# RomanJuranek/librectify

Hardware: AMD Instinct MI355X
Metric: Mpix/s end-to-end (detect+VP) on 4K frames, batch call of 64 frames, 5 in flight (higher is better)
Workload: dtype f32

## Files before the change

include/librectify_amd.h:

```cpp
#pragma once
#include <math.h>
#include <stddef.h>
#include <stdint.h>

#include "librectify.h"

#if defined(__GNUC__)
#pragma GCC visibility push(default)
#endif

#ifdef __cplusplus
using librectify::ImageTransform;
using librectify::LineSegment;
using librectify::Point;
using librectify::RectificationConfig;
extern "C" {
#endif

typedef struct lr_context lr_context;
enum lr_pixel_format { LR_PIX_U8 = 0, LR_PIX_U8X3 = 1, LR_PIX_F32 = 2 };

int lr_context_create(int device, lr_context** out);
void lr_context_destroy(lr_context* ctx);
void lr_release_thread_context(void);
// ... 349 lines not shown
int lr_stage_seeds(lr_context* ctx, int* n_seeds);
int lr_stage_flood(lr_context* ctx, int* n_components);
int lr_stage_fit(lr_context* ctx, LineSegment* out, int capacity, int* n_lines);

enum lr_buffer_id {
    LR_BUF_DX = 0,
    LR_BUF_DY = 1,
    LR_BUF_DMASK = 2,
    LR_BUF_LABEL = 3,
    LR_BUF_SEED_IDX = 4,
    LR_BUF_SEED_BIN = 5,
    LR_BUF_SEED_THR = 6,
    LR_BUF_MAXMAG = 7,
    LR_BUF_SEED_SIZE = 8,
    LR_BUF_SEED_REC = 9,
};
int lr_download(lr_context* ctx, int buffer_id, void* dst, size_t bytes);

enum lr_stage_id {
    LR_T_UPLOAD = 0,
    LR_T_FILTER = 1,
    LR_T_SEEDS = 2,
    LR_T_FLOOD = 3,
    LR_T_FIT = 4,
    LR_T_RANSAC = 5,
    LR_T_TOTAL = 6,
    LR_T_FILTER_KERNEL = 7,
    LR_T_COUNT = 8,
};
int lr_stage_times(lr_context* ctx, float* ms, int count);
// ... 33 lines not shown
```

librectify_amd/__init__.py:

```python
import collections
import ctypes as C
import os

import numpy as np

_HERE = os.path.dirname(os.path.abspath(__file__))
LIB_PATH = os.path.join(_HERE, "librectify_amd.so")

LINE_DTYPE = np.dtype(
    [("x1", "<f4"), ("y1", "<f4"), ("x2", "<f4"), ("y2", "<f4"), ("weight", "<f4"), ("err", "<f4"), ("group_id", "<i4")]
)


class Point(C.Structure):
    _fields_ = [("x", C.c_float), ("y", C.c_float), ("z", C.c_float)]


class ImageTransform(C.Structure):
    _fields_ = [
        ("width", C.c_int),
        ("height", C.c_int),
        ("top_left", Point),
        ("top_right", Point),
        ("bottom_left", Point),
# ... 30 lines not shown

class DrawLinesArgs(C.Structure):
    _fields_ = [("lines", C.c_void_p), ("n_lines", C.c_size_t), ("frames", C.c_void_p), ("H", C.c_void_p)]


class JpegArgs(C.Structure):
    _fields_ = [("frames", C.c_void_p), ("sizes", C.c_void_p)]


class JpegDecodeArgs(C.Structure):
    _fields_ = [("h_src", C.c_void_p), ("frames", C.c_void_p), ("info", C.c_void_p)]


BUF_DX, BUF_DY, BUF_DMASK, BUF_LABEL, BUF_SEED_IDX, BUF_SEED_BIN, BUF_SEED_THR, BUF_MAXMAG, BUF_SEED_SIZE = range(9)
BUF_SEED_REC = 9
T_UPLOAD, T_FILTER, T_SEEDS, T_FLOOD, T_FIT, T_RANSAC, T_TOTAL, T_FILTER_KERNEL, T_COUNT = range(9)
PIX_U8, PIX_U8X3, PIX_F32 = range(3)
WARP_PREPARE = 0x100
WARP_PACKED = 0x200
WARP_RAGGED = 0x800
WARP_LINES = 0x1000
JPEG_OPTIMIZE = 0x10
WARP_JPEG = 0x2000
WARP_CUBIC = 0x8000
JPEG_SCALED = 0x80000
JPEG_ANY_SAMPLING = 0x20000
WARP_JPEG_DECODE = 0x4000
WARP_BORDER = 0x40000
BORDER_CONSTANT, BORDER_REPLICATE, BORDER_REFLECT, BORDER_REFLECT_101 = 0, 1, 2, 4
WARP_LENS = 0x100000
# ... 912 lines not shown
        h, w = self.shape
        if buf in (BUF_DX, BUF_DY):
            a = np.zeros((h, w), np.float32)
        elif buf == BUF_DMASK:
            a = np.zeros((h, w), np.uint8)
        elif buf == BUF_LABEL:
            a = np.zeros((h, w), np.int32)
        elif buf in (BUF_SEED_IDX, BUF_SEED_BIN, BUF_SEED_SIZE):
            a = np.zeros(self.n_seeds, np.int32)
        elif buf == BUF_SEED_THR:
            a = np.zeros(self.n_seeds, np.float32)
        elif buf == BUF_MAXMAG:
            a = np.zeros(1, np.float32)
        elif buf == BUF_SEED_REC:
            a = np.zeros((self.n_seeds, 4), np.uint32)
        else:
            raise ValueError(buf)
        if a.nbytes:
            _check(lib().lr_download(self._h, buf, _ptr(a), a.nbytes))
        return a

    def stage_times(self):
        t = np.zeros(T_COUNT, np.float32)
        _check(lib().lr_stage_times(self._h, _ptr(t), T_COUNT))
        return t

    def stage_times_partial(self):
        ms = C.c_float(0)
        _check(lib().lr_filter_kernel_ms(self._h, C.byref(ms)))
        return ms.value
# ... 945 lines not shown
```

librectify_amd/csrc/api.cpp:

```cpp
#include <algorithm>
#include <cstdio>
#include <cstdlib>
#include <cstring>
#include <memory>
#include <new>
#include <stdexcept>
#include <string>

#include "context.h"
#include "host.h"

using namespace lramd;

namespace {

struct CtxDeleter {
    void operator()(lr_context* c) const { ctx_destroy(c); }
};

std::unique_ptr<lr_context, CtxDeleter>& thread_context_slot() {
    thread_local std::unique_ptr<lr_context, CtxDeleter> ctx;
    return ctx;
}

// ... 451 lines not shown
    try {
        const size_t npix = (size_t)ctx->w * ctx->h;
        const void* src = nullptr;
        size_t have = 0;
        switch (buffer_id) {
            case LR_BUF_DX: src = ctx->ws.dx; have = npix * 4; break;
            case LR_BUF_DY: src = ctx->ws.dy; have = npix * 4; break;
            case LR_BUF_DMASK: src = ctx->ws.dmask; have = npix; break;
            case LR_BUF_LABEL: src = ctx->ws.label; have = npix * 4; break;
            case LR_BUF_SEED_IDX: src = ctx->ws.seed_idx; have = (size_t)ctx->n_seeds * 4; break;
            case LR_BUF_SEED_BIN: src = ctx->ws.seed_bin; have = (size_t)ctx->n_seeds * 4; break;
            case LR_BUF_SEED_THR: src = ctx->ws.seed_thr; have = (size_t)ctx->n_seeds * 4; break;
            case LR_BUF_MAXMAG: src = ctx->maxmag; have = 4; break;
            case LR_BUF_SEED_SIZE: src = ctx->ws.seed_size; have = (size_t)ctx->n_seeds * 4; break;
            case LR_BUF_SEED_REC: src = ctx->ws.seed_rec; have = (size_t)ctx->n_seeds * 16; break;
            default: set_error("lr_download: unknown buffer id"); return 1;
        }
        if (buffer_id == LR_BUF_DMASK && ctx->dmask_consumed) {
            set_error("lr_download: LR_BUF_DMASK was consumed by lr_stage_flood (labelled pixels are cleared); download it after lr_stage_filter");
            return 1;
        }
        if (bytes > have) {
            set_error("lr_download: request larger than the buffer");
            return 1;
        }
        LR_HIP(hipSetDevice(ctx->device));
        LR_HIP(hipStreamSynchronize(ctx->stream));
        LR_HIP(hipMemcpy(dst, src, bytes, hipMemcpyDeviceToHost));
        return 0;
    } catch (...) {
// ... 83 lines not shown

int lr_refine_lines(lr_context* ctx, const LineSegment* in, int n, LineSegment* out, int* n_out) {
    try {
        std::vector<LineSegment> v(in, in + n);
        if (ctx_refine(ctx, v)) return 1;
        std::memcpy(out, v.data(), v.size() * sizeof(LineSegment));
        *n_out = (int)v.size();
        return 0;
    } catch (...) {
        return guard_fail("lr_refine_lines");
    }
}

void lr_set_estimator(lr_context* ctx, int kind, int param) {
    ctx->opt.estimator = kind;
    if (kind == 3) ctx->opt.cht_d = param > 0 ? param : 128;
    else ctx->opt.prosac_T_N = param;
}

int lr_estimate_line_pencils_cht(lr_context* ctx, LineSegment* lines, int n, int max_models, float inlier_deg,
                                 float garbage_deg, int d, float* models3, int* n_models, uint32_t* peak_cells,
                                 uint64_t* votes) {
    try {
        std::vector<LineSegment> v(lines, lines + n);
        ChtTrace tr;
        if (ctx_estimate_line_pencils_cht(ctx, v, max_models, inlier_deg, garbage_deg, d, &tr)) return 1;
        std::memcpy(lines, v.data(), sizeof(LineSegment) * (size_t)n);
        for (size_t k = 0; k < tr.models.size(); ++k) {
            if (models3) {
                models3[3 * k + 0] = tr.models[k].x;
// ... 87 lines not shown
```

librectify_amd/csrc/common.h:

```cpp
#pragma once
#include <hip/hip_runtime.h>

#include <cstdint>
#include <string>

#include "../../include/librectify_amd.h"

namespace lramd {

constexpr float kEps = 1e-6f;
constexpr int kMaxModels = 4;
constexpr int kMaxPeelModels = 5;
constexpr float kInlierDeg = 2.0f;
constexpr float kGarbageDeg = 4.0f;
constexpr int kRansacMaxIter = 10000;
constexpr int kEdgeKernelSize = 2;
constexpr float kEdgeKernelSigma = 1.0f;
constexpr int kSeedDist = 2;
constexpr float kSeedRatio = 0.95f;
constexpr float kTraceTolerance = 0.25f;
constexpr float kLineMaxErr = 2.0f;
constexpr float kLineMinLength = 5.f;
constexpr int kComponentMinSize = 5;
constexpr int kBins = 8;
// ... 186 lines not shown
    uint32_t scheduled = 0;
};
constexpr int kFloodCtrlWords = 56;
int flood_enqueue(const FloodBuffers& B, const FloodFrame& F, FloodProgress* P, uint32_t* h_ctrl, hipStream_t s);
int flood_finish(const FloodBuffers& B, const FloodFrame& F, FloodProgress* P, uint32_t* h_ctrl, int* rounds_out,
                 uint32_t* tiers_out ,
                 bool* extra, hipStream_t s);

size_t fit_temp_bytes(size_t max_pixels, uint32_t max_segments);
struct HugeSort {
    uint32_t* tab = nullptr;
    uint32_t* list = nullptr;
    uint32_t* jobs = nullptr;
    uint32_t max = 0;
};
int launch_component_offsets(const int32_t* seed_size, const uint32_t* d_n_seeds, uint32_t seed_cap, int min_size,
                             uint32_t* comp_rank, uint32_t* comp_seed, uint32_t* comp_off,
                             uint32_t* totals , uint32_t* large_list, uint32_t large_cap,
                             uint32_t* n_large, void* temp, size_t temp_bytes, uint32_t frame_tag, uint32_t* cursor, const HugeSort& hs,
                             hipStream_t s);
int launch_component_scatter(const uint32_t* label, size_t npix, const uint32_t* comp_rank, const uint32_t* comp_off,
                             uint32_t* cursor, uint32_t* px, const HugeSort& hs, uint32_t* n_large, bool with_huge, hipStream_t s);
int launch_component_sort(const uint32_t* px_in, uint32_t* px_out, const uint32_t* comp_off, const uint32_t* d_n_comp,
                          uint32_t comp_cap, const uint32_t* large_list, uint32_t large_cap, const uint32_t* n_large,
                          uint32_t* scratch, const uint32_t* cursor, const HugeSort& hs, bool with_huge, hipStream_t s);
int launch_fit(const uint32_t* px_sorted, const uint32_t* px_unsorted, const uint32_t* comp_off, const uint32_t* comp_seed, const uint32_t* d_n_comp,
               uint32_t comp_cap, const int32_t* seed_bin, const float* dx, const float* dy, int w, BinTrig trig,
               float* scratch_w, LineSegment* out, const uint32_t* cursor, const HugeSort& hs, const uint32_t* n_large, bool with_huge,
               hipStream_t s);

struct PencilSoA {
    const float* ax;
    const float* ay;
// ... 18 lines not shown
    float* len;
    float* hx;
    float* hy;
    float* hz;
    uint32_t* orig;
    PencilSoA soa() const { return PencilSoA{ax, ay, dx, dy, len, hx, hy, hz}; }
};
enum {
    kGcLines = 0,
    kGcRemaining = 1,
    kGcRound = 2,
    kGcActive = 3,
    kGcBestIter0 = 4,
    kGcWords = 8,
};
int launch_filter_lines(const LineSegment* raw, const uint32_t* d_n_raw, uint32_t raw_cap, float min_length,
                        LineSegment* out, uint32_t* gctl, float* gnorm, const PencilTable* all, const PencilTable* round0,
                        hipStream_t s);
int launch_lines_bbox(LineSegment* lines, uint32_t n, uint32_t* gctl, float* gnorm, hipStream_t s);
int launch_pencil_model(const LineSegment* lines, const uint32_t* gctl, const float* gnorm, PencilTable all,
                        PencilTable round0, uint32_t line_cap, hipStream_t s);
int launch_peel(PencilTable cur, PencilTable nxt, PencilTable all, unsigned long long* best_slots, uint64_t seed,
                float tol, float garbage_tol, int max_models, uint32_t* gctl, float* stage4 ,
                LineSegment* lines, float* models,
                const uint32_t* counts, uint32_t cap_lines, void* gather_block ,
                hipStream_t s);
int launch_cht_accumulate(PencilSoA m, uint32_t n, int d, unsigned long long* acc, hipStream_t s);
int launch_cht_votes(PencilSoA m, const uint32_t* idx, uint32_t n, int d, unsigned long long* acc, bool subtract,
                     unsigned long long* n_votes, hipStream_t s);
int launch_cht_peak(const unsigned long long* acc, int d, uint32_t* out3, hipStream_t s);
int launch_refine_pairs(const void* seg, uint32_t n, void* edges, uint32_t* n_edges, uint32_t cap, hipStream_t s);
// ... 10 lines not shown
```

librectify_amd/csrc/context.h:

```cpp
#pragma once
#include <atomic>
#include <functional>
#include <memory>
#include <mutex>
#include <vector>

#include "buffers.h"
#include "common.h"
#include "vp_host.h"

namespace lramd {
struct StagingCrew;

struct Settings {
    uint64_t ransac_seed = 0;
    int ransac_iters = kRansacMaxIter;
    int estimator = 0;
    int prosac_T_N = -1;
    int cht_d = 128;
    int batch_streams = 5;
    int flood_mode = 1;
    bool flood_giant_step = true;
    bool flood_jit = true;
    bool flood_partial = true;
    bool flood_log_sweep = false;
    bool flood_logs = true;
    bool flood_staged = false;
    bool timing_on = false;
};


struct Workspace {
    size_t cap_pix = 0;
    int cap_tiles = 0;
    DeviceBuffer<float> dx, dy;
    DeviceBuffer<uint8_t> dmask;
    DeviceBuffer<uint64_t> cand;
    DeviceBuffer<uint32_t> cand_count, tile_max;
    DeviceBuffer<uint32_t> tile_pass;
    DeviceBuffer<uint32_t> tile_off;
    DeviceBuffer<uint64_t> keys_a, keys_b;
    DeviceBuffer<int32_t> seed_idx, seed_bin;
// ... 254 lines not shown
```

librectify_amd/csrc/frame.hip:

```cpp
#include "host.h"

#include <cstdio>
#include <cstdlib>
#include <cstring>

namespace lramd {


namespace {

uint32_t round_up(uint32_t v, uint32_t m) { return (v + m - 1) / m * m; }

uint32_t initial_seed_cap(size_t npix) {
    return (uint32_t)std::min<size_t>(npix, std::max<size_t>(round_up((uint32_t)(npix / 32), 1024), 4096));
}

uint32_t line_cap_for(const lr_context* c) {
    return (uint32_t)std::min<size_t>(c->seed_cap, c->ws.cap_pix / 6 + 16);
}


PencilTable table_of(lr_context* c, int which) {
    const size_t cl = c->cap_glines;
    float* b = c->d_tables + (size_t)which * 8 * cl;
// ... 171 lines not shown
    c->flood_hold_hint = c->flood_tiers[3] != 0 && c->flood_tiers[8] >= 16;
    constexpr uint32_t kStagedKeep = 64;
    c->flood_staged_hint = c->flood_tiers[14] != 0 && (!c->flood_staged_hint || c->flood_tiers[0] >= kStagedKeep);
    c->flood_staged_streak = c->flood_staged_hint ? c->flood_staged_streak + 1 : 0;
    if (c->flood_staged_streak >= 16) {
        c->flood_staged_hint = false;
        c->flood_staged_streak = 0;
    }
    if (c->flood_staged_hint) c->flood_hold_hint = false;

    c->flood_rounds_hint = std::max(std::max(c->flood_rounds + 2, 6), c->flood_rounds_hint - 1);
    c->flood_rounds_last = c->flood_rounds;
    return 0;
}

int enqueue_fit(lr_context* c) {
    const size_t npix = (size_t)c->w * c->h;
    const uint32_t comp_cap = line_cap_for(c);
    const bool with_huge = !(c->opt.flood_mode != 0 && c->flood_prog.sizes_known && c->flood_prog.max_flood <= (1u << 14));
    if (launch_component_offsets(c->ws.seed_size, c->d_counts + kCntSeeds, c->seed_cap, kComponentMinSize, c->ws.comp_rank,
                                 c->ws.comp_seed, c->ws.comp_off, c->d_counts + kCntComp, c->ws.comp_large,
                                 (uint32_t)(c->ws.cap_pix / 64 + 16), c->d_counts + kCntLarge, c->ws.temp, c->ws.temp.cap(), ++c->fit_tag ? c->fit_tag : ++c->fit_tag, c->ws.cursor,
                                 with_huge ? c->ws.huge : HugeSort{}, c->stream))
        return 1;
    if (launch_component_scatter(c->ws.label, npix, c->ws.comp_rank, c->ws.comp_off, c->ws.cursor, c->ws.px_a, c->ws.huge, c->d_counts + kCntLarge, with_huge,
                                 c->stream))
        return 1;
    if (launch_component_sort(c->ws.px_a, c->ws.px_b, c->ws.comp_off, c->d_counts + kCntComp, comp_cap, c->ws.comp_large,
                              (uint32_t)(c->ws.cap_pix / 64 + 16), c->d_counts + kCntLarge, reinterpret_cast<uint32_t*>(c->ws.keys_b.get()),
                              c->ws.cursor, c->ws.huge, with_huge, c->stream))
        return 1;
    static const bool fit_debug = std::getenv("LIBRECTIFY_FIT_DEBUG") != nullptr;
    if (fit_debug) {
        uint32_t cnt[16];
        LR_HIP(hipStreamSynchronize(c->stream));
        LR_HIP(hipMemcpy(cnt, c->d_counts, sizeof(cnt), hipMemcpyDeviceToHost));
        std::fprintf(stderr, "fit: with_huge %d (sizes known %d, largest flood %u); seeds %u comps %u px %u; lists: %u of 65..1024 px, %u longer, %u huge in %u buckets; counter %u\n",
                     (int)with_huge, (int)c->flood_prog.sizes_known, c->flood_prog.max_flood, cnt[0], cnt[1], cnt[2], cnt[4], cnt[5], cnt[6], cnt[7], cnt[10]);
        const uint32_t nj = std::min<uint32_t>(cnt[7], 6);
        std::vector<uint32_t> jobs(4 * nj + 4);
        if (nj) LR_HIP(hipMemcpy(jobs.data(), c->ws.huge.jobs, nj * 16, hipMemcpyDeviceToHost));
        for (uint32_t j = 0; j < nj; ++j) std::fprintf(stderr, "   bucket job %u: start %u, %u px, table word %u\n", j, jobs[4 * j], jobs[4 * j + 1], jobs[4 * j + 2]);
    }
    if (launch_fit(c->ws.px_b, c->ws.px_a, c->ws.comp_off, c->ws.comp_seed, c->d_counts + kCntComp, comp_cap, c->ws.seed_bin, c->ws.dx, c->ws.dy, c->w,
                   c->trig, c->ws.scratch_w, c->ws.d_lines, c->ws.cursor, c->ws.huge, c->d_counts + kCntLarge, with_huge, c->stream))
        return 1;
    if (c->opt.timing_on) LR_HIP(hipEventRecord(c->ev[4], c->stream));
    return 0;
}

}

int enqueue_groups(lr_context* c, uint32_t line_cap, int max_models, float inlier_deg, float garbage_deg, int n_iter,
                   uint64_t seed, bool model_done, bool gather) {
    if (max_models > kMaxPeelModels) {
        set_error("estimate_line_pencils: max_models above " + std::to_string(kMaxPeelModels) + " (the reference uses 4, config.h:25)");
        return 1;
    }
    const float tol = cos_threshold(inlier_deg), garbage_tol = cos_threshold(garbage_deg);
// ... 23 lines not shown
    (void)hipEventElapsedTime(&ms, c->ev[0], c->ev[1]);
    c->stage_ms[LR_T_FILTER] = ms;
    c->stage_ms[LR_T_FILTER_KERNEL] = ms;
    (void)hipEventElapsedTime(&ms, c->ev[1], c->ev[2]);
    c->stage_ms[LR_T_SEEDS] = ms;
    (void)hipEventElapsedTime(&ms, c->ev[2], c->ev[3]);
    c->stage_ms[LR_T_FLOOD] = ms;
    (void)hipEventElapsedTime(&ms, c->ev[3], c->ev[4]);
    c->stage_ms[LR_T_FIT] = ms;
    if (with_groups) {
        (void)hipEventElapsedTime(&ms, c->ev[5], c->ev[6]);
        c->stage_ms[LR_T_RANSAC] = ms;
        (void)hipEventElapsedTime(&ms, c->ev[0], c->ev[6]);
        c->stage_ms[LR_T_TOTAL] = ms;
    }
}

void adapt_seed_cap(lr_context* c, uint32_t n_seeds) {
    const size_t npix = (size_t)c->w * c->h;
    if (n_seeds > c->seed_cap)
        c->seed_cap = (uint32_t)std::min<size_t>(npix, std::max<uint32_t>(4096, round_up(n_seeds * 2u, 1024)));
    else if (n_seeds < c->seed_cap / 3 || n_seeds > c->seed_cap / 5 * 4)
        c->seed_cap = (uint32_t)std::min<size_t>(npix, std::max<uint32_t>(4096, round_up(n_seeds + n_seeds / 2, 1024)));
}

}

struct TimingOn {
    lr_context* c;
    bool was;
// ... 68 lines not shown
    return 0;
}

int ctx_detect(lr_context* c, const float* d_image, int w, int h, int stride, std::vector<LineSegment>& raw) {
    if (ctx_stage_filter(c, d_image, w, h, stride)) return 1;
    if (ctx_stage_seeds(c)) return 1;
    if (ctx_stage_flood(c)) return 1;
    return ctx_stage_fit(c, raw);
}

int run_frame(lr_context* c, const void* d_image, int format, int w, int h, int stride, float min_length, bool refine,
              std::vector<LineSegment>& out, bool filter_enqueued) {
    out.clear();
    const double t_begin = now_ms();
    const bool fused = !refine && c->opt.estimator == 0;
    const int n_iter = c->opt.ransac_iters;
    auto groups_after_fit = [&]() -> int {
        const uint32_t lc = line_cap_for(c);
        if (ensure_group_capacity(c, lc)) return 1;
        if (ensure_result_block(c, std::max<size_t>(c->res_lines_cap, 4096))) return 1;
        if (c->opt.timing_on) LR_HIP(hipEventRecord(c->ev[5], c->stream));
        const PencilTable all = table_of(c, 0), round0 = table_of(c, 1);
        if (launch_filter_lines(c->ws.d_lines, c->d_counts + kCntComp, lc, min_length, c->d_flines, c->d_gctl, c->d_gnorm, &all, &round0,
                                c->stream))
            return 1;
        static_assert(kMaxModels >= 1 && kGcWords == 8 && kResHeaderBytes == 256, "the last peeling round carries the result block (peel_kernel)");
        if (enqueue_groups(c, lc, kMaxModels, kInlierDeg, kGarbageDeg, n_iter, c->opt.ransac_seed, true, true)) return 1;
        if (c->opt.timing_on) LR_HIP(hipEventRecord(c->ev[6], c->stream));
        return 0;
    };
    auto after_fit = [&]() -> int {
        if (fused) return groups_after_fit();
        LR_HIP(hipMemcpyAsync(c->h_counts, c->d_counts, 8 * sizeof(uint32_t), hipMemcpyDeviceToHost, c->stream));
        return 0;
    };
    c->frame_laps = 0;
    for (int attempt = 0;; ++attempt) {
        c->frame_laps += 1;
        if (!(filter_enqueued && attempt == 0) && enqueue_filter(c, d_image, format, w, h, stride)) return 1;
        if (enqueue_seeds(c)) return 1;
        if (enqueue_flood(c)) return 1;
        if (enqueue_fit(c)) return 1;
        if (after_fit()) return 1;
        const double t_enq = now_ms();
        const double t_pre = now_ms();
        if (c->sleep_in_wait) {
            LR_HIP(hipEventRecord(c->ev_wait, c->stream));
            LR_HIP(hipEventSynchronize(c->ev_wait));
        } else {
            LR_HIP(hipStreamSynchronize(c->stream));
        }
        c->host_ms[0] = t_enq - t_begin;
        c->host_ms[1] = t_pre - t_enq;
        c->host_ms[2] = now_ms() - t_pre;
        const uint32_t* cnt = fused ? reinterpret_cast<const uint32_t*>(c->h_res.get()) : c->h_counts.get();
        c->n_seeds = cnt[kCntSeeds];
        if (c->n_seeds <= c->seed_cap) break;
        if (attempt > 0) {
            set_error("seed count exceeds the sort capacity twice");
            return 1;
        }
        adapt_seed_cap(c, c->n_seeds);
    }
    bool extra = false;
    if (finish_flood(c, &extra)) return 1;
    if (extra) {
        c->frame_laps += 1;
        if (enqueue_fit(c)) return 1;
        if (after_fit()) return 1;
        LR_HIP(hipStreamSynchronize(c->stream));
    }
    const uint32_t* cnt = fused ? reinterpret_cast<const uint32_t*>(c->h_res.get()) : c->h_counts.get();
    c->n_comp = cnt[kCntComp];
    c->n_px = cnt[kCntPx];
    adapt_seed_cap(c, c->n_seeds);
    c->stage_valid[0] = c->stage_valid[1] = false;
    c->stage_valid[2] = c->stage_valid[3] = true;
    if (fused) {
        const uint32_t* gctl = reinterpret_cast<const uint32_t*>(c->h_res + 32);
        const size_t n = gctl[kGcLines];
        out.resize(n);
        const size_t have = std::min<size_t>(n, c->res_lines_cap);
        if (have) std::memcpy(out.data(), c->h_res + kResHeaderBytes, have * sizeof(LineSegment));
        if (n > have) {
            LR_HIP(hipMemcpyAsync(out.data() + have, c->d_flines + have, (n - have) * sizeof(LineSegment),
                                  hipMemcpyDeviceToHost, c->stream));
            LR_HIP(hipStreamSynchronize(c->stream));
            if (ensure_result_block(c, round_up((uint32_t)(n + n / 2), 1024))) return 1;
        }
        record_stage_times(c, true);
#ifdef LR_PEEL_TIMING
        {
// ... 180 lines not shown
```

librectify_amd/csrc/host.h:

```cpp
#pragma once
#include <atomic>
#include <chrono>
#include <condition_variable>
#include <mutex>
#include <string>
#include <thread>
#include <vector>

#include "context.h"
#include "reg_plan.h"

namespace lramd {

inline double now_ms() {
    return std::chrono::duration<double, std::milli>(std::chrono::steady_clock::now().time_since_epoch()).count();
}

struct JoinedThreads {
    std::vector<std::thread> th;
    void join() {
        for (auto& t : th)
            if (t.joinable()) t.join();
    }
    ~JoinedThreads() { join(); }
};

enum { kCntSeeds = 0, kCntComp = 1, kCntPx = 2, kCntLarge = 4 };

int ensure_flood_buffers(lr_context* c);
int ensure_group_capacity(lr_context* c, size_t n_lines);

int enqueue_groups(lr_context* c, uint32_t line_cap, int max_models, float inlier_deg, float garbage_deg, int n_iter,
                   uint64_t seed, bool model_done = false, bool gather = false);
int run_frame(lr_context* c, const void* d_image, int format, int w, int h, int stride, float min_length, bool refine,
              std::vector<LineSegment>& out, bool filter_enqueued = false);

int ensure_copy_stream(lr_context* c);
bool is_page_locked(const void* p);
int staging_threads(int num_threads, size_t frame_bytes = 0);
void bind_this_thread_near(int device);
int upload_rows(lr_context* c, void* dst, void* stage, const void* buffer, int w, int h, int stride, int bpp, int num_threads,
                hipStream_t up);
// ... 95 lines not shown
```

librectify_amd/csrc/kernels_fit.hip:

```cpp
#include <algorithm>
#include <cstring>

#include <atomic>

#include "common.h"

namespace lramd {
namespace {

constexpr uint32_t kNoComp = 0xFFFFFFFFu;

constexpr uint32_t kSortLds = 1024;
constexpr uint32_t kSortLdsBig = 16384;
constexpr uint32_t kHugeShift = 14;
constexpr uint32_t kHugeFlag = 0x80000000u;
constexpr int kOffPer = 8;
constexpr uint32_t kOffChunk = 256 * kOffPer;

__device__ __forceinline__ void chunk_counts(const int32_t* __restrict__ seed_size, uint32_t n_seeds, int min_size,
                                             uint32_t k0, int (&sz)[kOffPer], uint32_t& c, uint32_t& p) {
    c = p = 0;
#pragma unroll
    for (int j = 0; j < kOffPer; ++j) {
        sz[j] = (k0 + j < n_seeds) ? seed_size[k0 + j] : 0;
        if (sz[j] > min_size) {
            c += 1u;
            p += (uint32_t)sz[j];
        }
    }
}

__global__ __launch_bounds__(256) void component_offsets_kernel(const int32_t* __restrict__ seed_size,
                                                                const uint32_t* __restrict__ n_ptr, uint32_t cap,
                                                                int min_size, unsigned long long* __restrict__ status, uint32_t tag,
                                                                uint32_t* __restrict__ comp_rank,
                                                                uint32_t* __restrict__ comp_seed,
                                                                uint32_t* __restrict__ comp_off,
                                                                uint32_t* __restrict__ totals,
                                                                uint32_t* __restrict__ large_list,
                                                                uint32_t large_cap, uint32_t* __restrict__ n_large,
                                                                uint32_t* __restrict__ cursor, uint32_t* __restrict__ huge_list,
                                                                uint32_t huge_max) {
    __shared__ uint32_t s_c[4], s_p[4], s_cc[4], s_cp[4];
    const uint32_t n_seeds = min(*n_ptr, cap);
    const int tid = threadIdx.x, lane = tid & 63, wv = tid >> 6;
    const uint32_t k0 = blockIdx.x * kOffChunk + (uint32_t)tid * kOffPer;
    int sz[kOffPer];
    uint32_t c, p;
    chunk_counts(seed_size, n_seeds, min_size, k0, sz, c, p);
    uint32_t ic = c, ip = p;
#pragma unroll
    for (int off = 1; off < 64; off <<= 1) {
        const uint32_t tc = (uint32_t)__shfl_up((int)ic, off);
        const uint32_t tp = (uint32_t)__shfl_up((int)ip, off);
        if (lane >= off) {
            ic += tc;
            ip += tp;
        }
    }
    if (lane == 63) {
        s_c[wv] = ic;
        s_p[wv] = ip;
    }
    __syncthreads();
    if (tid == 0) {
        const unsigned long long t = (unsigned long long)tag << 32;
        const unsigned long long wc = t | (unsigned long long)(s_c[0] + s_c[1] + s_c[2] + s_c[3]);
        const unsigned long long wp = t | (unsigned long long)(s_p[0] + s_p[1] + s_p[2] + s_p[3]);
        if (blockIdx.x == 0) {
#pragma unroll
            for (int i = 0; i < 4; ++i) __hip_atomic_store(&n_large[i], 0u, __ATOMIC_RELAXED, __HIP_MEMORY_SCOPE_AGENT);
            __hip_atomic_store(&status[0], wc, __ATOMIC_RELEASE, __HIP_MEMORY_SCOPE_AGENT);
            __hip_atomic_store(&status[1], wp, __ATOMIC_RELEASE, __HIP_MEMORY_SCOPE_AGENT);
        } else {
            __hip_atomic_store(&status[2u * blockIdx.x], wc, __ATOMIC_RELAXED, __HIP_MEMORY_SCOPE_AGENT);
            __hip_atomic_store(&status[2u * blockIdx.x + 1u], wp, __ATOMIC_RELAXED, __HIP_MEMORY_SCOPE_AGENT);
        }
    }
    uint32_t cc = 0, cp = 0;
    for (uint32_t i = (uint32_t)tid; i < blockIdx.x; i += 256) {
        unsigned long long wc = 0ull, wp = 0ull;
        for (uint32_t spins = 0; spins < (1u << 22); ++spins) {
            wc = __hip_atomic_load(&status[2u * i], __ATOMIC_RELAXED, __HIP_MEMORY_SCOPE_AGENT);
            wp = __hip_atomic_load(&status[2u * i + 1u], __ATOMIC_RELAXED, __HIP_MEMORY_SCOPE_AGENT);
            if ((uint32_t)(wc >> 32) == tag && (uint32_t)(wp >> 32) == tag) break;
            __builtin_amdgcn_s_sleep(2);
        }
        cc += (uint32_t)wc;
        cp += (uint32_t)wp;
    }
#pragma unroll
    for (int off = 32; off >= 1; off >>= 1) {
        cc += (uint32_t)__shfl_xor((int)cc, off);
        cp += (uint32_t)__shfl_xor((int)cp, off);
    }
    if (lane == 0) {
        s_cc[wv] = cc;
        s_cp[wv] = cp;
    }
    __syncthreads();
    uint32_t rank = s_cc[0] + s_cc[1] + s_cc[2] + s_cc[3] + ic - c;
    uint32_t off_px = s_cp[0] + s_cp[1] + s_cp[2] + s_cp[3] + ip - p;
    for (int i = 0; i < wv; ++i) {
        rank += s_c[i];
        off_px += s_p[i];
    }
#pragma unroll
    for (int j = 0; j < kOffPer; ++j) {
        const uint32_t k = k0 + j;
        if (k < n_seeds) {
            const bool keep = sz[j] > min_size;
            comp_rank[k] = keep ? rank : kNoComp;
            if (keep) {
                comp_seed[rank] = k;
                comp_off[rank] = off_px;
                if (sz[j] > (int)kSortLds) large_list[large_cap - 1u - atomicAdd(n_large + 1, 1u)] = rank;
                else if (sz[j] > 64) large_list[atomicAdd(n_large, 1u)] = rank;
                uint32_t cur = 0u;
                if (sz[j] > (int)kSortLdsBig && huge_max != 0u) {
                    const uint32_t hi = atomicAdd(n_large + 2, 1u);
                    if (hi < huge_max) {
                        cur = hi | kHugeFlag;
                        huge_list[hi] = rank;
                    }
                }
                cursor[rank] = cur;
                rank += 1u;
                off_px += (uint32_t)sz[j];
            }
        }
    }
    if (blockIdx.x == gridDim.x - 1 && tid == 255) {
        totals[0] = rank;
        totals[1] = off_px;
        comp_off[rank] = off_px;
    }
}

__global__ __launch_bounds__(256) void component_scatter_kernel(const uint32_t* __restrict__ label, size_t npix,
                                                                const uint32_t* __restrict__ comp_rank,
                                                                const uint32_t* __restrict__ comp_off,
                                                                uint32_t* __restrict__ cursor,
                                                                uint32_t* __restrict__ px, uint32_t* __restrict__ huge_tab,
                                                                uint32_t nb) {
    const int lane = threadIdx.x & 63;
    const size_t step = (size_t)gridDim.x * 256;
    const size_t n_pad = (npix + 255) / 256 * 256;
    constexpr int kU = 4;
    for (size_t i0 = (size_t)blockIdx.x * 256 + threadIdx.x; i0 < n_pad; i0 += step * kU) {
// ... 625 lines not shown
        l.y2 = a_r + d_r * t1;
        l.weight = S / (float)n;
        l.err = esum / (float)n;
        l.group_id = -1;
        out[comp] = l;
    }
}

}

size_t fit_temp_bytes(size_t max_pixels, uint32_t max_segments) {
    (void)max_segments;
    return (max_pixels / kOffChunk + 2) * 2 * sizeof(unsigned long long) + 256;
}

int launch_component_offsets(const int32_t* seed_size, const uint32_t* d_n_seeds, uint32_t seed_cap, int min_size,
                             uint32_t* comp_rank, uint32_t* comp_seed, uint32_t* comp_off, uint32_t* totals,
                             uint32_t* large_list, uint32_t large_cap, uint32_t* n_large, void* temp, size_t temp_bytes,
                             uint32_t frame_tag, uint32_t* cursor, const HugeSort& hs, hipStream_t s) {
    const uint32_t chunks = (seed_cap + kOffChunk - 1) / kOffChunk;
    if (chunks == 0 || temp_bytes < (size_t)chunks * 2 * sizeof(unsigned long long)) {
        set_error("launch_component_offsets: workspace too small");
        return 1;
    }
    hipLaunchKernelGGL(component_offsets_kernel, dim3(chunks), dim3(256), 0, s, seed_size, d_n_seeds, seed_cap, min_size,
                       static_cast<unsigned long long*>(temp), frame_tag, comp_rank, comp_seed, comp_off, totals, large_list, large_cap,
                       n_large, cursor, hs.list, hs.tab ? hs.max : 0u);
    LR_HIP(hipGetLastError());
    return 0;
}

int launch_component_scatter(const uint32_t* label, size_t npix, const uint32_t* comp_rank, const uint32_t* comp_off,
                             uint32_t* cursor, uint32_t* px, const HugeSort& hs, uint32_t* n_large, bool with_huge, hipStream_t s) {
    const uint32_t nb = (uint32_t)((npix + ((size_t)1 << kHugeShift) - 1) >> kHugeShift);
    const size_t want = (npix + 255) / 256;
    if (with_huge && hs.tab)
        hipLaunchKernelGGL(huge_count_kernel, dim3((unsigned)std::min<size_t>(want, 2048)), dim3(256), 0, s, label, npix, comp_rank, comp_off,
                           cursor, hs.tab, nb, hs.list, hs.max, reinterpret_cast<uint4*>(hs.jobs), n_large);
    const int blocks = (int)(want < 8192 ? want : 8192);
    hipLaunchKernelGGL(component_scatter_kernel, dim3(blocks > 0 ? blocks : 1), dim3(256), 0, s, label, npix, comp_rank,
                       comp_off, cursor, px, hs.tab, nb);
// ... 47 lines not shown
```

librectify_amd/csrc/kernels_groups.hip:

```cpp
#include "common.h"

namespace lramd {
namespace {

constexpr int kWG = 1024;
constexpr int kWaves = kWG / 64;

__device__ __forceinline__ float wave_tree(float v) {
#pragma unroll
    for (int off = 32; off >= 1; off >>= 1) v = v + __shfl_xor(v, off);
    return v;
}

__device__ __forceinline__ uint32_t block_rank(bool flag, uint32_t* s_cnt, uint32_t& total) {
    const int lane = threadIdx.x & 63, wv = threadIdx.x >> 6;
    const uint64_t m = __ballot(flag);
    __syncthreads();
    if (lane == 0) s_cnt[wv] = (uint32_t)__popcll(m);
    __syncthreads();
    uint32_t before = 0, tot = 0;
#pragma unroll
    for (int i = 0; i < kWaves; ++i) {
        const uint32_t c = s_cnt[i];
        before += i < wv ? c : 0u;
// ... 13 lines not shown
        hx = hx / nn;
        hy = hy / nn;
        hz = hz / nn;
    }
    const float ax = (x2 + x1) / 2, ay = (y2 + y1) / 2;
    const float dx = x2 - x1, dy = y2 - y1;
    const float len = sqrtf(dx * dx + dy * dy);
    const float ux = dx / len, uy = dy / len;
    all.ax[i] = ax; all.ay[i] = ay; all.dx[i] = ux; all.dy[i] = uy; all.len[i] = len;
    all.hx[i] = hx; all.hy[i] = hy; all.hz[i] = hz; all.orig[i] = i;
    round0.ax[i] = ax; round0.ay[i] = ay; round0.dx[i] = ux; round0.dy[i] = uy; round0.len[i] = len;
    round0.hx[i] = hx; round0.hy[i] = hy; round0.hz[i] = hz; round0.orig[i] = i;
}

__global__ __launch_bounds__(kWG) void filter_lines_kernel(const LineSegment* __restrict__ raw,
                                                           const uint32_t* __restrict__ n_raw_ptr, uint32_t raw_cap,
                                                           float min_length, LineSegment* __restrict__ out,
                                                           uint32_t* __restrict__ gctl, float* __restrict__ gnorm,
                                                           PencilTable all, PencilTable round0, uint32_t with_model) {
    constexpr int kFlB = 8;
    __shared__ uint32_t s_cnt[kFlB][kWaves];
    __shared__ float s_red[4][kWaves];
    const uint32_t n_raw = min(*n_raw_ptr, raw_cap);
    const float ml = fmaxf(min_length, kLineMinLength);
    const int lane = threadIdx.x & 63, wv = threadIdx.x >> 6;
    uint32_t base = 0;
    if (n_raw >= 2u) {
        for (uint32_t i0 = 0; i0 < n_raw; i0 += kWG * kFlB) {
            LineSegment l[kFlB];
            uint64_t m[kFlB];
#pragma unroll
            for (int b = 0; b < kFlB; ++b) {
                const uint32_t i = i0 + (uint32_t)b * kWG + threadIdx.x;
                l[b] = LineSegment{};
                if (i < n_raw) l[b] = raw[i];
            }
#pragma unroll
            for (int b = 0; b < kFlB; ++b) {
                const uint32_t i = i0 + (uint32_t)b * kWG + threadIdx.x;
                const float dx = l[b].x2 - l[b].x1, dy = l[b].y2 - l[b].y1;
                const bool keep = i < n_raw && sqrtf(dx * dx + dy * dy) > ml && l[b].err < kLineMaxErr;
                m[b] = __ballot(keep);
// ... 366 lines not shown
    peel_body(cur, nxt, all, best_slots, seed, tol, garbage_tol, max_models, gctl, stage_g, lines, models);
    if (gather_dst == nullptr) return;
    __syncthreads();
    const uint32_t t = threadIdx.x;
    const uint32_t* gw = gctl;
    if (t < 8) gather_dst[t] = counts[t];
    else if (t < 16) gather_dst[t] = gw[t - 8];
    else if (t < 56) gather_dst[t] = reinterpret_cast<const uint32_t*>(models)[t - 16];
    const uint32_t n = min(gw[kGcLines], cap_lines) * (uint32_t)(sizeof(LineSegment) / 4);
    const uint32_t* lw = reinterpret_cast<const uint32_t*>(lines);
    for (uint32_t i = t; i < n; i += kWG) gather_dst[64 + i] = lw[i];
}

}

int launch_filter_lines(const LineSegment* raw, const uint32_t* d_n_raw, uint32_t raw_cap, float min_length,
                        LineSegment* out, uint32_t* gctl, float* gnorm, const PencilTable* all, const PencilTable* round0,
                        hipStream_t s) {
    const bool with_model = all != nullptr && round0 != nullptr;
    hipLaunchKernelGGL(filter_lines_kernel, dim3(1), dim3(kWG), 0, s, raw, d_n_raw, raw_cap, min_length, out, gctl, gnorm,
                       with_model ? *all : PencilTable{}, with_model ? *round0 : PencilTable{}, with_model ? 1u : 0u);
    LR_HIP(hipGetLastError());
    return 0;
}

int launch_lines_bbox(LineSegment* lines, uint32_t n, uint32_t* gctl, float* gnorm, hipStream_t s) {
    hipLaunchKernelGGL(lines_bbox_kernel, dim3(1), dim3(kWG), 0, s, lines, n, gctl, gnorm);
    LR_HIP(hipGetLastError());
    return 0;
}

int launch_pencil_model(const LineSegment* lines, const uint32_t* gctl, const float* gnorm, PencilTable all,
                        PencilTable round0, uint32_t line_cap, hipStream_t s) {
    if (line_cap == 0) return 0;
    hipLaunchKernelGGL(pencil_model_kernel, dim3((line_cap + 255) / 256), dim3(256), 0, s, lines, gctl, gnorm, all, round0);
// ... 16 lines not shown
```

Baseline: 10630.

## Skip fitting components too small to yield lines above the minimum length

Adds a fit threshold derived from min_length: on the fused detect+VP path, components whose pixel count cannot produce a segment longer than min_length are left out of scatter, sort and fit. The offsets kernel still reports the full component counts through atomics, and the fit-only counts go to new counter slots that the sort, fit and filter kernels now read. This cuts per-component fit and sort work. The exchange is an extra pass of atomic counting, plus reliance on the bound that segment length never exceeds the pixel count times 1.4157.

```diff
diff --git a/include/librectify_amd.h b/include/librectify_amd.h
--- a/include/librectify_amd.h
+++ b/include/librectify_amd.h
@@ -387,6 +387,7 @@
     LR_BUF_MAXMAG = 7,
     LR_BUF_SEED_SIZE = 8,
     LR_BUF_SEED_REC = 9,
+    LR_BUF_COUNTS = 10,
 };
 int lr_download(lr_context* ctx, int buffer_id, void* dst, size_t bytes);
 
diff --git a/librectify_amd/__init__.py b/librectify_amd/__init__.py
--- a/librectify_amd/__init__.py
+++ b/librectify_amd/__init__.py
@@ -68,6 +68,7 @@
 
 BUF_DX, BUF_DY, BUF_DMASK, BUF_LABEL, BUF_SEED_IDX, BUF_SEED_BIN, BUF_SEED_THR, BUF_MAXMAG, BUF_SEED_SIZE = range(9)
 BUF_SEED_REC = 9
+BUF_COUNTS = 10
 T_UPLOAD, T_FILTER, T_SEEDS, T_FLOOD, T_FIT, T_RANSAC, T_TOTAL, T_FILTER_KERNEL, T_COUNT = range(9)
 PIX_U8, PIX_U8X3, PIX_F32 = range(3)
 WARP_PREPARE = 0x100
@@ -1010,6 +1011,8 @@
             a = np.zeros(1, np.float32)
         elif buf == BUF_SEED_REC:
             a = np.zeros((self.n_seeds, 4), np.uint32)
+        elif buf == BUF_COUNTS:
+            a = np.zeros(16, np.uint32)
         else:
             raise ValueError(buf)
         if a.nbytes:
diff --git a/librectify_amd/csrc/api.cpp b/librectify_amd/csrc/api.cpp
--- a/librectify_amd/csrc/api.cpp
+++ b/librectify_amd/csrc/api.cpp
@@ -489,6 +489,7 @@
             case LR_BUF_MAXMAG: src = ctx->maxmag; have = 4; break;
             case LR_BUF_SEED_SIZE: src = ctx->ws.seed_size; have = (size_t)ctx->n_seeds * 4; break;
             case LR_BUF_SEED_REC: src = ctx->ws.seed_rec; have = (size_t)ctx->n_seeds * 16; break;
+            case LR_BUF_COUNTS: src = ctx->d_counts; have = 16 * 4; break;
             default: set_error("lr_download: unknown buffer id"); return 1;
         }
         if (buffer_id == LR_BUF_DMASK && ctx->dmask_consumed) {
@@ -602,6 +603,7 @@
 
 void lr_set_estimator(lr_context* ctx, int kind, int param) {
     ctx->opt.estimator = kind;
+    if (kind == 0) ctx->opt.fit_prune = param != 0;
     if (kind == 3) ctx->opt.cht_d = param > 0 ? param : 128;
     else ctx->opt.prosac_T_N = param;
 }
diff --git a/librectify_amd/csrc/common.h b/librectify_amd/csrc/common.h
--- a/librectify_amd/csrc/common.h
+++ b/librectify_amd/csrc/common.h
@@ -224,9 +224,10 @@
     uint32_t* jobs = nullptr;
     uint32_t max = 0;
 };
-int launch_component_offsets(const int32_t* seed_size, const uint32_t* d_n_seeds, uint32_t seed_cap, int min_size,
+int launch_component_offsets(const int32_t* seed_size, const uint32_t* d_n_seeds, uint32_t seed_cap, int min_size, int fit_min,
                              uint32_t* comp_rank, uint32_t* comp_seed, uint32_t* comp_off,
-                             uint32_t* totals , uint32_t* large_list, uint32_t large_cap,
+                             uint32_t* totals , uint32_t* fit_totals ,
+                             uint32_t* large_list, uint32_t large_cap,
                              uint32_t* n_large, void* temp, size_t temp_bytes, uint32_t frame_tag, uint32_t* cursor, const HugeSort& hs,
                              hipStream_t s);
 int launch_component_scatter(const uint32_t* label, size_t npix, const uint32_t* comp_rank, const uint32_t* comp_off,
@@ -275,7 +276,7 @@
     kGcBestIter0 = 4,
     kGcWords = 8,
 };
-int launch_filter_lines(const LineSegment* raw, const uint32_t* d_n_raw, uint32_t raw_cap, float min_length,
+int launch_filter_lines(const LineSegment* raw, const uint32_t* d_n_fit, const uint32_t* d_n_raw, uint32_t raw_cap, float min_length,
                         LineSegment* out, uint32_t* gctl, float* gnorm, const PencilTable* all, const PencilTable* round0,
                         hipStream_t s);
 int launch_lines_bbox(LineSegment* lines, uint32_t n, uint32_t* gctl, float* gnorm, hipStream_t s);
diff --git a/librectify_amd/csrc/context.h b/librectify_amd/csrc/context.h
--- a/librectify_amd/csrc/context.h
+++ b/librectify_amd/csrc/context.h
@@ -26,6 +26,7 @@
     bool flood_log_sweep = false;
     bool flood_logs = true;
     bool flood_staged = false;
+    bool fit_prune = true;
     bool timing_on = false;
 };
 
diff --git a/librectify_amd/csrc/frame.hip b/librectify_amd/csrc/frame.hip
--- a/librectify_amd/csrc/frame.hip
+++ b/librectify_amd/csrc/frame.hip
@@ -1,5 +1,6 @@
 #include "host.h"
 
+#include <cmath>
 #include <cstdio>
 #include <cstdlib>
 #include <cstring>
@@ -209,19 +210,25 @@
     return 0;
 }
 
-int enqueue_fit(lr_context* c) {
+int fit_min_for(float min_length) {
+    const double ml = std::fmax((double)min_length, (double)kLineMinLength);
+    const double n = std::floor(ml / 1.4157);
+    return (int)std::min(std::max(n, (double)kComponentMinSize), 1073741824.0);
+}
+
+int enqueue_fit(lr_context* c, int fit_min = kComponentMinSize) {
     const size_t npix = (size_t)c->w * c->h;
     const uint32_t comp_cap = line_cap_for(c);
     const bool with_huge = !(c->opt.flood_mode != 0 && c->flood_prog.sizes_known && c->flood_prog.max_flood <= (1u << 14));
-    if (launch_component_offsets(c->ws.seed_size, c->d_counts + kCntSeeds, c->seed_cap, kComponentMinSize, c->ws.comp_rank,
-                                 c->ws.comp_seed, c->ws.comp_off, c->d_counts + kCntComp, c->ws.comp_large,
+    if (launch_component_offsets(c->ws.seed_size, c->d_counts + kCntSeeds, c->seed_cap, kComponentMinSize, fit_min, c->ws.comp_rank,
+                                 c->ws.comp_seed, c->ws.comp_off, c->d_counts + kCntComp, c->d_counts + kCntFitComp, c->ws.comp_large,
                                  (uint32_t)(c->ws.cap_pix / 64 + 16), c->d_counts + kCntLarge, c->ws.temp, c->ws.temp.cap(), ++c->fit_tag ? c->fit_tag : ++c->fit_tag, c->ws.cursor,
                                  with_huge ? c->ws.huge : HugeSort{}, c->stream))
         return 1;
     if (launch_component_scatter(c->ws.label, npix, c->ws.comp_rank, c->ws.comp_off, c->ws.cursor, c->ws.px_a, c->ws.huge, c->d_counts + kCntLarge, with_huge,
                                  c->stream))
         return 1;
-    if (launch_component_sort(c->ws.px_a, c->ws.px_b, c->ws.comp_off, c->d_counts + kCntComp, comp_cap, c->ws.comp_large,
+    if (launch_component_sort(c->ws.px_a, c->ws.px_b, c->ws.comp_off, c->d_counts + kCntFitComp, comp_cap, c->ws.comp_large,
                               (uint32_t)(c->ws.cap_pix / 64 + 16), c->d_counts + kCntLarge, reinterpret_cast<uint32_t*>(c->ws.keys_b.get()),
                               c->ws.cursor, c->ws.huge, with_huge, c->stream))
         return 1;
@@ -230,6 +237,7 @@
         uint32_t cnt[16];
         LR_HIP(hipStreamSynchronize(c->stream));
         LR_HIP(hipMemcpy(cnt, c->d_counts, sizeof(cnt), hipMemcpyDeviceToHost));
+        std::fprintf(stderr, "fit: threshold %d, %u components of %u px fitted\n", fit_min, cnt[kCntFitComp], cnt[kCntFitPx]);
         std::fprintf(stderr, "fit: with_huge %d (sizes known %d, largest flood %u); seeds %u comps %u px %u; lists: %u of 65..1024 px, %u longer, %u huge in %u buckets; counter %u\n",
                      (int)with_huge, (int)c->flood_prog.sizes_known, c->flood_prog.max_flood, cnt[0], cnt[1], cnt[2], cnt[4], cnt[5], cnt[6], cnt[7], cnt[10]);
         const uint32_t nj = std::min<uint32_t>(cnt[7], 6);
@@ -237,7 +245,7 @@
         if (nj) LR_HIP(hipMemcpy(jobs.data(), c->ws.huge.jobs, nj * 16, hipMemcpyDeviceToHost));
         for (uint32_t j = 0; j < nj; ++j) std::fprintf(stderr, "   bucket job %u: start %u, %u px, table word %u\n", j, jobs[4 * j], jobs[4 * j + 1], jobs[4 * j + 2]);
     }
-    if (launch_fit(c->ws.px_b, c->ws.px_a, c->ws.comp_off, c->ws.comp_seed, c->d_counts + kCntComp, comp_cap, c->ws.seed_bin, c->ws.dx, c->ws.dy, c->w,
+    if (launch_fit(c->ws.px_b, c->ws.px_a, c->ws.comp_off, c->ws.comp_seed, c->d_counts + kCntFitComp, comp_cap, c->ws.seed_bin, c->ws.dx, c->ws.dy, c->w,
                    c->trig, c->ws.scratch_w, c->ws.d_lines, c->ws.cursor, c->ws.huge, c->d_counts + kCntLarge, with_huge, c->stream))
         return 1;
     if (c->opt.timing_on) LR_HIP(hipEventRecord(c->ev[4], c->stream));
@@ -291,6 +299,7 @@
         (void)hipEventElapsedTime(&ms, c->ev[0], c->ev[6]);
         c->stage_ms[LR_T_TOTAL] = ms;
     }
+    (void)hipGetLastError();
 }
 
 void adapt_seed_cap(lr_context* c, uint32_t n_seeds) {
@@ -389,6 +398,7 @@
     out.clear();
     const double t_begin = now_ms();
     const bool fused = !refine && c->opt.estimator == 0;
+    const int fit_min = fused && c->opt.fit_prune ? fit_min_for(min_length) : kComponentMinSize;
     const int n_iter = c->opt.ransac_iters;
     auto groups_after_fit = [&]() -> int {
         const uint32_t lc = line_cap_for(c);
@@ -396,7 +406,7 @@
         if (ensure_result_block(c, std::max<size_t>(c->res_lines_cap, 4096))) return 1;
         if (c->opt.timing_on) LR_HIP(hipEventRecord(c->ev[5], c->stream));
         const PencilTable all = table_of(c, 0), round0 = table_of(c, 1);
-        if (launch_filter_lines(c->ws.d_lines, c->d_counts + kCntComp, lc, min_length, c->d_flines, c->d_gctl, c->d_gnorm, &all, &round0,
+        if (launch_filter_lines(c->ws.d_lines, c->d_counts + kCntFitComp, c->d_counts + kCntComp, lc, min_length, c->d_flines, c->d_gctl, c->d_gnorm, &all, &round0,
                                 c->stream))
             return 1;
         static_assert(kMaxModels >= 1 && kGcWords == 8 && kResHeaderBytes == 256, "the last peeling round carries the result block (peel_kernel)");
@@ -415,7 +425,7 @@
         if (!(filter_enqueued && attempt == 0) && enqueue_filter(c, d_image, format, w, h, stride)) return 1;
         if (enqueue_seeds(c)) return 1;
         if (enqueue_flood(c)) return 1;
-        if (enqueue_fit(c)) return 1;
+        if (enqueue_fit(c, fit_min)) return 1;
         if (after_fit()) return 1;
         const double t_enq = now_ms();
         const double t_pre = now_ms();
@@ -441,7 +451,7 @@
     if (finish_flood(c, &extra)) return 1;
     if (extra) {
         c->frame_laps += 1;
-        if (enqueue_fit(c)) return 1;
+        if (enqueue_fit(c, fit_min)) return 1;
         if (after_fit()) return 1;
         LR_HIP(hipStreamSynchronize(c->stream));
     }
@@ -450,7 +460,8 @@
     c->n_px = cnt[kCntPx];
     adapt_seed_cap(c, c->n_seeds);
     c->stage_valid[0] = c->stage_valid[1] = false;
-    c->stage_valid[2] = c->stage_valid[3] = true;
+    c->stage_valid[2] = true;
+    c->stage_valid[3] = fit_min == kComponentMinSize;
     if (fused) {
         const uint32_t* gctl = reinterpret_cast<const uint32_t*>(c->h_res + 32);
         const size_t n = gctl[kGcLines];
diff --git a/librectify_amd/csrc/host.h b/librectify_amd/csrc/host.h
--- a/librectify_amd/csrc/host.h
+++ b/librectify_amd/csrc/host.h
@@ -25,7 +25,7 @@
     ~JoinedThreads() { join(); }
 };
 
-enum { kCntSeeds = 0, kCntComp = 1, kCntPx = 2, kCntLarge = 4 };
+enum { kCntSeeds = 0, kCntComp = 1, kCntPx = 2, kCntLarge = 4, kCntFitComp = 12, kCntFitPx = 13 };
 
 int ensure_flood_buffers(lr_context* c);
 int ensure_group_capacity(lr_context* c, size_t n_lines);
diff --git a/librectify_amd/csrc/kernels_fit.hip b/librectify_amd/csrc/kernels_fit.hip
--- a/librectify_amd/csrc/kernels_fit.hip
+++ b/librectify_amd/csrc/kernels_fit.hip
@@ -17,13 +17,17 @@
 constexpr int kOffPer = 8;
 constexpr uint32_t kOffChunk = 256 * kOffPer;
 
-__device__ __forceinline__ void chunk_counts(const int32_t* __restrict__ seed_size, uint32_t n_seeds, int min_size,
-                                             uint32_t k0, int (&sz)[kOffPer], uint32_t& c, uint32_t& p) {
-    c = p = 0;
+__device__ __forceinline__ void chunk_counts(const int32_t* __restrict__ seed_size, uint32_t n_seeds, int min_size, int fit_min,
+                                             uint32_t k0, int (&sz)[kOffPer], uint32_t& c, uint32_t& p, uint32_t& rc, uint32_t& rp) {
+    c = p = rc = rp = 0;
 #pragma unroll
     for (int j = 0; j < kOffPer; ++j) {
         sz[j] = (k0 + j < n_seeds) ? seed_size[k0 + j] : 0;
         if (sz[j] > min_size) {
+            rc += 1u;
+            rp += (uint32_t)sz[j];
+        }
+        if (sz[j] > fit_min) {
             c += 1u;
             p += (uint32_t)sz[j];
         }
@@ -32,22 +36,22 @@
 
 __global__ __launch_bounds__(256) void component_offsets_kernel(const int32_t* __restrict__ seed_size,
                                                                 const uint32_t* __restrict__ n_ptr, uint32_t cap,
-                                                                int min_size, unsigned long long* __restrict__ status, uint32_t tag,
+                                                                int min_size, int fit_min, unsigned long long* __restrict__ status, uint32_t tag,
                                                                 uint32_t* __restrict__ comp_rank,
                                                                 uint32_t* __restrict__ comp_seed,
                                                                 uint32_t* __restrict__ comp_off,
-                                                                uint32_t* __restrict__ totals,
+                                                                uint32_t* __restrict__ totals, uint32_t* __restrict__ fit_totals,
                                                                 uint32_t* __restrict__ large_list,
                                                                 uint32_t large_cap, uint32_t* __restrict__ n_large,
                                                                 uint32_t* __restrict__ cursor, uint32_t* __restrict__ huge_list,
                                                                 uint32_t huge_max) {
-    __shared__ uint32_t s_c[4], s_p[4], s_cc[4], s_cp[4];
+    __shared__ uint32_t s_c[4], s_p[4], s_cc[4], s_cp[4], s_rc[4], s_rp[4];
     const uint32_t n_seeds = min(*n_ptr, cap);
     const int tid = threadIdx.x, lane = tid & 63, wv = tid >> 6;
     const uint32_t k0 = blockIdx.x * kOffChunk + (uint32_t)tid * kOffPer;
     int sz[kOffPer];
-    uint32_t c, p;
-    chunk_counts(seed_size, n_seeds, min_size, k0, sz, c, p);
+    uint32_t c, p, rc, rp;
+    chunk_counts(seed_size, n_seeds, min_size, fit_min, k0, sz, c, p, rc, rp);
     uint32_t ic = c, ip = p;
 #pragma unroll
     for (int off = 1; off < 64; off <<= 1) {
@@ -58,9 +62,16 @@
             ip += tp;
         }
     }
+#pragma unroll
+    for (int off = 32; off >= 1; off >>= 1) {
+        rc += (uint32_t)__shfl_xor((int)rc, off);
+        rp += (uint32_t)__shfl_xor((int)rp, off);
+    }
     if (lane == 63) {
         s_c[wv] = ic;
         s_p[wv] = ip;
+        s_rc[wv] = rc;
+        s_rp[wv] = rp;
     }
     __syncthreads();
     if (tid == 0) {
@@ -70,6 +81,8 @@
         if (blockIdx.x == 0) {
 #pragma unroll
             for (int i = 0; i < 4; ++i) __hip_atomic_store(&n_large[i], 0u, __ATOMIC_RELAXED, __HIP_MEMORY_SCOPE_AGENT);
+            __hip_atomic_store(&totals[0], 0u, __ATOMIC_RELAXED, __HIP_MEMORY_SCOPE_AGENT);
+            __hip_atomic_store(&totals[1], 0u, __ATOMIC_RELAXED, __HIP_MEMORY_SCOPE_AGENT);
             __hip_atomic_store(&status[0], wc, __ATOMIC_RELEASE, __HIP_MEMORY_SCOPE_AGENT);
             __hip_atomic_store(&status[1], wp, __ATOMIC_RELEASE, __HIP_MEMORY_SCOPE_AGENT);
         } else {
@@ -99,6 +112,13 @@
         s_cp[wv] = cp;
     }
     __syncthreads();
+    if (tid == 0) {
+        const uint32_t wrc = s_rc[0] + s_rc[1] + s_rc[2] + s_rc[3], wrp = s_rp[0] + s_rp[1] + s_rp[2] + s_rp[3];
+        if (wrc != 0u) {
+            __hip_atomic_fetch_add(&totals[0], wrc, __ATOMIC_RELAXED, __HIP_MEMORY_SCOPE_AGENT);
+            __hip_atomic_fetch_add(&totals[1], wrp, __ATOMIC_RELAXED, __HIP_MEMORY_SCOPE_AGENT);
+        }
+    }
     uint32_t rank = s_cc[0] + s_cc[1] + s_cc[2] + s_cc[3] + ic - c;
     uint32_t off_px = s_cp[0] + s_cp[1] + s_cp[2] + s_cp[3] + ip - p;
     for (int i = 0; i < wv; ++i) {
@@ -109,7 +129,7 @@
     for (int j = 0; j < kOffPer; ++j) {
         const uint32_t k = k0 + j;
         if (k < n_seeds) {
-            const bool keep = sz[j] > min_size;
+            const bool keep = sz[j] > fit_min;
             comp_rank[k] = keep ? rank : kNoComp;
             if (keep) {
                 comp_seed[rank] = k;
@@ -131,8 +151,8 @@
         }
     }
     if (blockIdx.x == gridDim.x - 1 && tid == 255) {
-        totals[0] = rank;
-        totals[1] = off_px;
+        fit_totals[0] = rank;
+        fit_totals[1] = off_px;
         comp_off[rank] = off_px;
     }
 }
@@ -788,8 +808,8 @@
     return (max_pixels / kOffChunk + 2) * 2 * sizeof(unsigned long long) + 256;
 }
 
-int launch_component_offsets(const int32_t* seed_size, const uint32_t* d_n_seeds, uint32_t seed_cap, int min_size,
-                             uint32_t* comp_rank, uint32_t* comp_seed, uint32_t* comp_off, uint32_t* totals,
+int launch_component_offsets(const int32_t* seed_size, const uint32_t* d_n_seeds, uint32_t seed_cap, int min_size, int fit_min,
+                             uint32_t* comp_rank, uint32_t* comp_seed, uint32_t* comp_off, uint32_t* totals, uint32_t* fit_totals,
                              uint32_t* large_list, uint32_t large_cap, uint32_t* n_large, void* temp, size_t temp_bytes,
                              uint32_t frame_tag, uint32_t* cursor, const HugeSort& hs, hipStream_t s) {
     const uint32_t chunks = (seed_cap + kOffChunk - 1) / kOffChunk;
@@ -797,8 +817,12 @@
         set_error("launch_component_offsets: workspace too small");
         return 1;
     }
-    hipLaunchKernelGGL(component_offsets_kernel, dim3(chunks), dim3(256), 0, s, seed_size, d_n_seeds, seed_cap, min_size,
-                       static_cast<unsigned long long*>(temp), frame_tag, comp_rank, comp_seed, comp_off, totals, large_list, large_cap,
+    if (fit_min < min_size) {
+        set_error("launch_component_offsets: fit threshold below the size threshold");
+        return 1;
+    }
+    hipLaunchKernelGGL(component_offsets_kernel, dim3(chunks), dim3(256), 0, s, seed_size, d_n_seeds, seed_cap, min_size, fit_min,
+                       static_cast<unsigned long long*>(temp), frame_tag, comp_rank, comp_seed, comp_off, totals, fit_totals, large_list, large_cap,
                        n_large, cursor, hs.list, hs.tab ? hs.max : 0u);
     LR_HIP(hipGetLastError());
     return 0;
diff --git a/librectify_amd/csrc/kernels_groups.hip b/librectify_amd/csrc/kernels_groups.hip
--- a/librectify_amd/csrc/kernels_groups.hip
+++ b/librectify_amd/csrc/kernels_groups.hip
@@ -51,18 +51,20 @@
 }
 
 __global__ __launch_bounds__(kWG) void filter_lines_kernel(const LineSegment* __restrict__ raw,
-                                                           const uint32_t* __restrict__ n_raw_ptr, uint32_t raw_cap,
+                                                           const uint32_t* __restrict__ n_fit_ptr,
+                                                           const uint32_t* __restrict__ n_all_ptr, uint32_t raw_cap,
                                                            float min_length, LineSegment* __restrict__ out,
                                                            uint32_t* __restrict__ gctl, float* __restrict__ gnorm,
                                                            PencilTable all, PencilTable round0, uint32_t with_model) {
     constexpr int kFlB = 8;
     __shared__ uint32_t s_cnt[kFlB][kWaves];
     __shared__ float s_red[4][kWaves];
-    const uint32_t n_raw = min(*n_raw_ptr, raw_cap);
+    const uint32_t n_raw = min(*n_fit_ptr, raw_cap);
+    const uint32_t n_all = min(*n_all_ptr, raw_cap);
     const float ml = fmaxf(min_length, kLineMinLength);
     const int lane = threadIdx.x & 63, wv = threadIdx.x >> 6;
     uint32_t base = 0;
-    if (n_raw >= 2u) {
+    if (n_all >= 2u) {
         for (uint32_t i0 = 0; i0 < n_raw; i0 += kWG * kFlB) {
             LineSegment l[kFlB];
             uint64_t m[kFlB];
@@ -459,11 +461,11 @@
 
 }
 
-int launch_filter_lines(const LineSegment* raw, const uint32_t* d_n_raw, uint32_t raw_cap, float min_length,
+int launch_filter_lines(const LineSegment* raw, const uint32_t* d_n_fit, const uint32_t* d_n_raw, uint32_t raw_cap, float min_length,
                         LineSegment* out, uint32_t* gctl, float* gnorm, const PencilTable* all, const PencilTable* round0,
                         hipStream_t s) {
     const bool with_model = all != nullptr && round0 != nullptr;
-    hipLaunchKernelGGL(filter_lines_kernel, dim3(1), dim3(kWG), 0, s, raw, d_n_raw, raw_cap, min_length, out, gctl, gnorm,
+    hipLaunchKernelGGL(filter_lines_kernel, dim3(1), dim3(kWG), 0, s, raw, d_n_fit, d_n_raw, raw_cap, min_length, out, gctl, gnorm,
                        with_model ? *all : PencilTable{}, with_model ? *round0 : PencilTable{}, with_model ? 1u : 0u);
     LR_HIP(hipGetLastError());
     return 0;
```

Measured after the change: 10860 (median of 6 runs). +2.2%, better.
